# Amandaynzhou/MMT-PSM

Hardware: AMD Instinct MI355X
Metric: imgs/sec (student+teacher step, 1000x1000, AUG_K=2) (higher is better)
Workload: dtype f32

## Files before the change

### include/mmtpsm.h

```cpp
#ifndef MMTPSM_H
#define MMTPSM_H
#include <stdint.h>
#ifdef __cplusplus
extern "C" {
#endif

#define MMT_EINVAL (-22)

int mmt_version(void);

typedef struct {
  const float* feat[4];
  float* grad_feat[4];
  int H[4];
  int W[4];
  float scale[4];
  int num_levels;
  int N;
  int C;
} mmt_pyramid;

int mmt_roi_align_forward(const mmt_pyramid* pyr , const float* rois, const int32_t* levels,
                          int K, int PH, int PW, int sampling_ratio, float* out, void* stream);
int mmt_roi_align_forward_bf16(const mmt_pyramid* pyr , const float* rois, const int32_t* levels,
// ... 132 lines not shown
} mmt_conv_args;

int mmt_conv_forward(const mmt_conv_args* a , void* stream);
enum { MMT_ENTRY_LIB = 0, MMT_ENTRY_F16 = 1 };
enum { MMT_ASSUME_X = 1, MMT_ASSUME_W = 2, MMT_ASSUME_W_PLANES = 4, MMT_ASSUME_X_PLANES = 8, MMT_ASSUME_F16_SCALARS = 16 };
enum {
  MMT_ROUTE_NONE = 0,
  MMT_ROUTE_FP32 = 1,
  MMT_ROUTE_SPLIT = 2,
  MMT_ROUTE_DMA = 3,
  MMT_ROUTE_DMA_BF16X = 4,
  MMT_ROUTE_ROWS = 5,
  MMT_ROUTE_STRIP = 6,
  MMT_ROUTE_PG = 7,
  MMT_ROUTE_C64 = 8
};
enum { MMT_X_AS_IS = 0, MMT_X_BF16_PLANES = 1, MMT_X_F16_PLANES = 2 };
typedef struct {
  int family;
  int tag;
  int bm, bn;
  int kgroups;
  int panels;
  int ksplit;
  int strip_tw, strip_ksplit, strip_korder;
  int pg_rows, pg_ksplit;
  int wanted;
  int x_form;
  int writes_rb;
  int switches;
} mmt_conv_route_t;
int mmt_conv_route(const mmt_conv_args* a , int entry, int assume, mmt_conv_route_t* out );
enum { MMT_SW_SPLITK = 1, MMT_SW_STRIP = 2, MMT_SW_ROWS = 4, MMT_SW_PG = 8, MMT_SW_C64 = 16, MMT_SW_DIRECT_EPI = 32 };
int mmt_conv_switches(void);
int mmt_set_conv_precision(int mode);
int mmt_amax(const float* x, long n, const float* rowscale, long inner, int rows, float* amax , void* stream);
int mmt_amax_stats(const float* x, long n, float* slot , void* stream);
int mmt_sum_stats(const float* a, const float* b, const float* c, const float* d, float* y, long n,
                  float* slot , void* stream);
int mmt_stats_combine(const float* const* slots , int n, float* out , void* stream);
int mmt_split_planes_f16(const float* x, void* planes, long plane_stride, long n, float scale, const float* amax ,
                         float* scale_out , float* amax_next ,
                         float* zero_slot , void* stream);
int mmt_pack_weight_f16(const float* w, void* planes, long plane_stride, int Cout, int K, float scale, const float* amax,
                        float* scale_out, void* stream);
int mmt_pack_weight_flipped_f16(const float* w, const float* scale, void* planes, long plane_stride, int Cout, int KH, int KW,
                                int Cin, const float* amax, float* scale_out, void* stream);
int mmt_conv3x3_strip_f16x2(const mmt_conv_args* a , const float* s_x , const float* s_w , void* stream);
int mmt_conv_forward_f16x2(const mmt_conv_args* a , const float* x_amax , const float* s_w , void* stream);
int mmt_get_conv_precision(void);
int mmt_stem_fused(const float* x, int N, int H, int W, const float* w_s2d, const void* w_planes, long w_plane_stride,
                   const float* s_w , const float* scale, const float* shift, const float* x_slot , float* y,
                   float* y_slot , void* stream);
int mmt_c64_conv3_fused(const float* x, int N, int H, int W, const float* w2, const void* w2_planes, long w2_plane_stride,
                        const float* s_w2 , const float* scale2, const float* shift2, const float* x_slot ,
                        const float* w3, const void* w3_planes, long w3_plane_stride, const float* s_w3 , const float* scale3,
                        const float* shift3, const float* res, float* out, float* out_slot ,
                        const float* o2_scale , int o2_scale_is_amax, float* o2_amax_next ,
                        float* out_amax_next , const float* w1, const void* w1_planes, long w1_plane_stride,
                        const float* s_w1 , const float* scale1, const float* shift1, const float* out_scale ,
                        float* o1_next, float* o1_next_slot , void* stream);
int mmt_conv_wgrad_planes_splits(const mmt_conv_args* a );
int mmt_conv_wgrad_planes(const mmt_conv_args* a , const float* dy, const void* x_planes, long x_plane_stride,
                          const void* dy_planes, long dy_plane_stride, const float* s_x, const float* s_dy, const float* rowscale,
                          float* dw, float* dbias, float* workspace, void* stream);
typedef struct {
  void* fn;
  long a[16];
} mmt_call;
int mmt_replay(const mmt_call* calls , int n, int* failed_index );
int mmt_split_planes_f16_rb(const float* x, void* planes, long plane_stride, int rows, int W, int C, const float* amax,
                            float* scale_out, void* stream);
typedef struct mmt_wgrad_job {
  mmt_conv_args a;
  const float* dy; const float* rowscale; float* dw; float* dbias;
  const void* x_planes; long x_plane_stride; const void* dy_planes; long dy_plane_stride; const float* s_x; const float* s_dy;
} mmt_wgrad_job;
int mmt_conv_wgrad_group_workspace(const mmt_wgrad_job* jobs , int n, long* floats_out );
int mmt_conv_wgrad_group(const mmt_wgrad_job* jobs , int n, float* workspace, long workspace_floats, void* stream);
int mmt_sum_stats_rb(const float* a, const float* b, const float* c, const float* d, float* y, int rows, int W, int C, float* slot,
                     void* planes, long plane_stride, const float* scale, float* amax_next, void* stream);
int mmt_rb_scales_update(float* state, int n, void* stream);
int mmt_conv_forward_pg(const mmt_conv_args* a , const float* s_x , const float* s_w , int tile_rows,
                        int ksplit, void* stream);
typedef struct { long src_off, dst_off; int Cout, K, unit0, pad; } mmt_pack_desc;
long mmt_packed_weight_elems(int Cout, int K);
int mmt_pack_weight(const float* w, void* planes, long plane_stride, int Cout, int K, void* stream);
int mmt_pack_weight_flipped(const float* w, const float* scale, void* planes, long plane_stride, int Cout, int KH, int KW,
                            int Cin, void* stream);
int mmt_split_planes(const float* x, void* planes, long plane_stride, long n, void* stream);
typedef struct { const float* w; const float* scale; void* dst; long plane_stride; int Cout, KH, KW, Cin, unit0, pad; } mmt_flip_desc;
int mmt_pack_weights_flipped(const mmt_flip_desc* descs , const int* unit_desc , int n_units, void* stream);
int mmt_pack_weights(const float* base, void* planes, long plane_stride, const mmt_pack_desc* descs ,
                     const int* unit_desc , int n_units, void* stream);
int mmt_pack_weights_f16(const float* base, void* planes, long plane_stride, const mmt_pack_desc* descs ,
                         const int* unit_desc , int n_units, int n_descs, float* stat , void* stream);
int mmt_pack_weights_flipped_f16(const mmt_flip_desc* descs , const int* unit_desc , int n_units, int n_descs,
                                 float* stat , void* stream);

int mmt_conv_wgrad_splits(const mmt_conv_args* a );
int mmt_conv_wgrad(const mmt_conv_args* a , const float* dy,
                   const float* rowscale , float* dw, float* dbias ,
                   float* workspace , void* stream);

int mmt_colsum(const float* dy, int M, int C, float* out, void* stream);

// ... 116 lines not shown
```

### mmt-psm_amd/csrc/conv_stem.hip

```cpp
#include "conv_shared.h"

namespace {

struct StemP {
  const float* x;
  const unsigned short* wpl; long wpl_stride;
  const float* w;
  const float* scale; const float* shift;
  float* y;
  const float* x_slot;
  const float* s_w;
  unsigned* amax_out; int amax_stats;
  int N, H, W, Hc, Wc, Hp, Wp, tiles_y, tiles_x;
};

constexpr int SPH = 19, SPW = 35, SPIX = SPH * SPW;
constexpr int SPL = 672 * 32;
constexpr int SB_OFF = 2 * SPL;
constexpr int STEM_LDS = 128 * 1024;

__device__ __forceinline__ float stem_exact(const StemP& p, int n, int oy, int ox, int co) {
  float acc = 0.f;
  for (int a = 0; a < 4; a++)
    for (int b = 0; b < 4; b++) {
      const int si = oy - 2 + a, sj = ox - 2 + b;
      if ((unsigned)si >= (unsigned)p.Hc || (unsigned)sj >= (unsigned)p.Wc) continue;
      for (int ch = 0; ch < 16; ch++) {
        const int c = ch & 3;
        if (c == 3) continue;
        const float xv = p.x[(((long)n * 3 + c) * p.H + 2 * si + (ch >> 3)) * p.W + 2 * sj + ((ch >> 2) & 1)];
        acc = fmaf(xv, p.w[((co * 4 + a) * 4 + b) * 16 + ch], acc);
      }
    }
  return acc;
}

__global__ __launch_bounds__(512) void stem_fused_kernel(const StemP p) {
  extern __shared__ __attribute__((aligned(16))) float lds[];
  char* const sm = (char*)lds;
  const int tid = threadIdx.x, lane = tid & 63;
  const int wave = __builtin_amdgcn_readfirstlane(tid >> 6);
  int bid = blockIdx.x;
  const int tx = bid % p.tiles_x; bid /= p.tiles_x;
  const int ty = bid % p.tiles_y;
  const int n = bid / p.tiles_y;
  const int py0 = ty * 7, px0 = tx * 15;
  const int oy0 = 2 * py0 - 1, ox0 = 2 * px0 - 1;
  const int sy0 = oy0 - 2, sx0 = ox0 - 2;
  const F16Guard guard = f16_guard_load(p.x_slot);
  const float sx = f16_scale_of(*p.x_slot);

  if (f16_guard_bad(guard)) {
    float amx = 0.f;
    for (int o = tid; o < 7 * 15 * 64; o += 512) {
      const int co = o & 63, q = (o >> 6) % 15, j = (o >> 6) / 15;
      const int py = py0 + j, px = px0 + q;
      if (py >= p.Hp || px >= p.Wp) continue;
      float m = 0.f;
      for (int dy = -1; dy <= 1; dy++)
        for (int dx = -1; dx <= 1; dx++) {
          const int oy = 2 * py + dy, ox = 2 * px + dx;
          if ((unsigned)oy >= (unsigned)p.Hc || (unsigned)ox >= (unsigned)p.Wc) continue;
          m = fmaxf(m, fmaxf(stem_exact(p, n, oy, ox, co) * p.scale[co] + p.shift[co], 0.f));
        }
      p.y[(((long)n * p.Hp + py) * p.Wp + px) * 64 + co] = m;
      amx = fmaxf(amx, m);
    }
    if (p.amax_out && amx > 0.f) atomicMax(p.amax_out, __builtin_bit_cast(unsigned, amx));
    return;
  }

  {
    const __amdgpu_buffer_rsrc_t rs_b = __builtin_amdgcn_make_buffer_rsrc((void*)p.wpl, 0, 0x7ffffff0, 0x00020000);
#pragma unroll
    for (int i = 0; i < 8; i++) {
      const int item = wave + 8 * i, q = item >> 5, rest = item & 31;
      __builtin_amdgcn_raw_ptr_buffer_load_lds(rs_b, (lds_ptr_t)(sm + SB_OFF + item * 1024), 16,
                                               (int)((q * p.wpl_stride + (long)rest * 512 + lane * 8) * 2), 0, 0, 0);
    }
  }
  typedef float f32x2 __attribute__((ext_vector_type(2)));
#pragma unroll
  for (int rnd = 0; rnd < 3; rnd++) {
    const int item = tid + 512 * rnd;
    if (item < 2 * SPIX) {
      const int pix = item >> 1, bh = item & 1;
      const int pr = pix / SPW, pc = pix - pr * SPW;
      const int si = sy0 + pr, sj = sx0 + pc;
      f32x2 v[3];
      const bool ok = (unsigned)si < (unsigned)p.Hc && (unsigned)sj < (unsigned)p.Wc;
#pragma unroll
      for (int c = 0; c < 3; c++)
        v[c] = ok ? *(const f32x2*)(p.x + (((long)n * 3 + c) * p.H + 2 * si + bh) * p.W + 2 * sj) : f32x2{0.f, 0.f};
      uint2 o0[2], o1[2];
      split4h(f32x4{v[0][0], v[1][0], v[2][0], 0.f}, sx, o0);
      split4h(f32x4{v[0][1], v[1][1], v[2][1], 0.f}, sx, o1);
      char* const dst = sm + pix * 32 + ((bh ^ (pix >> 3)) & 1) * 16;
      *(uint4*)dst = uint4{o0[0].x, o0[0].y, o1[0].x, o1[0].y};
      *(uint4*)(dst + SPL) = uint4{o0[1].x, o0[1].y, o1[1].x, o1[1].y};
    }
  }
  asm volatile("s_waitcnt vmcnt(0) lgkmcnt(0)" ::: "memory");
  __syncthreads();

  const int lr = lane & 31, kh2 = lane >> 5;
  const int boff = SB_OFF + lr * 32 + (((kh2 ^ (lr >> 3)) & 1) << 4);
  auto a_addr = [&](int a, int ta, int tb) {
    const int pidx = (2 * wave + a + ta) * SPW + lr + tb;
    return pidx * 32 + (((kh2 ^ (pidx >> 3)) & 1) << 4);
  };
  f32x16 acc[2][2];
#pragma unroll
  for (int a = 0; a < 2; a++)
#pragma unroll
    for (int b = 0; b < 2; b++)
#pragma unroll
      for (int r = 0; r < 16; r++) acc[a][b][r] = 0.f;
  auto fread = [&](int s, f16x8 (&fa)[2][2], f16x8 (&fb)[2][2]) {
    const int ta = s >> 2, tb = s & 3;
#pragma unroll
    for (int a = 0; a < 2; a++) {
      const int ad = a_addr(a, ta, tb);
      fa[0][a] = *(const f16x8*)(sm + ad);
      fa[1][a] = *(const f16x8*)(sm + ad + SPL);
    }
#pragma unroll
    for (int q = 0; q < 2; q++)
#pragma unroll
      for (int b = 0; b < 2; b++) fb[q][b] = *(const f16x8*)(sm + boff + ((q * 16 + s) * 2 + b) * 1024);
  };
  auto mma = [&](const f16x8 (&fa)[2][2], const f16x8 (&fb)[2][2]) {
#pragma unroll
    for (int pr = 0; pr < 3; pr++) {
      const int qa = pr == 1 ? 1 : 0, qb = pr == 0 ? 1 : 0;
#pragma unroll
      for (int a = 0; a < 2; a++)
#pragma unroll
        for (int b = 0; b < 2; b++)
          acc[a][b] = __builtin_amdgcn_mfma_f32_32x32x16_f16(fa[qa][a], fb[qb][b], acc[a][b], 0, 0, 0);
    }
  };
  {
    f16x8 faP[2][2], fbP[2][2], faQ[2][2], fbQ[2][2];
    fread(0, faP, fbP);
#pragma unroll
    for (int s = 0; s < 16; s += 2) {
      fread(s + 1, faQ, fbQ);
      mma(faP, fbP);
      if (s + 2 < 16) fread(s + 2, faP, fbP);
      mma(faQ, fbQ);
    }
  }
  __syncthreads();

  const int col_l = lane & 31, rq = lane >> 5;
  const float inv = 1.f / (sx * *p.s_w);
  float sc[2], sh[2];
#pragma unroll
  for (int b = 0; b < 2; b++) { sc[b] = p.scale[b * 32 + col_l] * inv; sh[b] = p.shift[b * 32 + col_l]; }
  f32x16 m01[2];
#pragma unroll
  for (int b = 0; b < 2; b++)
#pragma unroll
    for (int r = 0; r < 16; r++) {
      const int ox = ox0 + 8 * (r >> 2) + (r & 3) + 4 * rq;
      const bool cok = (unsigned)ox < (unsigned)p.Wc;
      float v[2];
#pragma unroll
      for (int a = 0; a < 2; a++) {
        const int oy = oy0 + 2 * wave + a;
        const float t = fmaxf(acc[a][b][r] * sc[b] + sh[b], 0.f);
        v[a] = (cok && (unsigned)oy < (unsigned)p.Hc) ? t : 0.f;
      }
      acc[0][b][r] = v[0];
      m01[b][r] = fmaxf(v[0], v[1]);
    }
  float* const xr = lds;
  float* const hv = lds + 8 * 32 * 64;
#pragma unroll
  for (int b = 0; b < 2; b++)
#pragma unroll
    for (int r = 0; r < 16; r++)
      xr[(wave * 32 + 8 * (r >> 2) + (r & 3) + 4 * rq) * 64 + b * 32 + col_l] = acc[0][b][r];
  __syncthreads();
  if (wave < 7) {
#pragma unroll
    for (int b = 0; b < 2; b++)
#pragma unroll
      for (int r = 0; r < 16; r++) {
        const int col = 8 * (r >> 2) + (r & 3) + 4 * rq;
        hv[(wave * 32 + col) * 64 + b * 32 + col_l] = fmaxf(m01[b][r], xr[((wave + 1) * 32 + col) * 64 + b * 32 + col_l]);
      }
  }
  __syncthreads();
  float amx = 0.f, asum = 0.f, acnt = 0.f;
  for (int o = tid; o < 7 * 15 * 16; o += 512) {
    const int c4 = o & 15, q = (o >> 4) % 15, j = (o >> 4) / 15;
    const int py = py0 + j, px = px0 + q;
    if (py >= p.Hp || px >= p.Wp) continue;
    const f32x4* const row = (const f32x4*)(hv + (j * 32 + 2 * q) * 64) + c4;
    const f32x4 t0 = row[0], t1 = row[16], t2 = row[32];
    f32x4 m;
#pragma unroll
    for (int e = 0; e < 4; e++) {
      m[e] = fmaxf(fmaxf(t0[e], t1[e]), t2[e]);
      amx = fmaxf(amx, m[e]);
      asum += m[e];
    }
    acnt += 4.f;
    *(f32x4*)(p.y + (((long)n * p.Hp + py) * p.Wp + px) * 64 + c4 * 4) = m;
  }
  if (p.amax_out) {
    __syncthreads();
    float* const red = lds;
    const bool stats = p.amax_stats && (blockIdx.x & 63) == 0;
#pragma unroll
    for (int o = 32; o > 0; o >>= 1) amx = fmaxf(amx, __shfl_xor(amx, o, 64));
    if (stats) {
#pragma unroll
      for (int o = 32; o > 0; o >>= 1) { asum += __shfl_xor(asum, o, 64); acnt += __shfl_xor(acnt, o, 64); }
    }
    if (lane == 0) { red[wave] = amx; red[16 + wave] = asum; red[32 + wave] = acnt; }
    __syncthreads();
    if (tid == 0) {
      float m = red[0], sm_ = red[16], cn = red[32];
      for (int i = 1; i < 8; i++) { m = fmaxf(m, red[i]); sm_ += red[16 + i]; cn += red[32 + i]; }
      const unsigned bits = __builtin_bit_cast(unsigned, m);
      if (m > 0.f && bits > __hip_atomic_load(p.amax_out, __ATOMIC_RELAXED, __HIP_MEMORY_SCOPE_AGENT)) atomicMax(p.amax_out, bits);
      if (stats && cn > 0.f) {
        const int k = (blockIdx.x >> 6) & 15;
        atomicAdd((float*)p.amax_out + 1 + k, sm_);
        atomicAdd((float*)p.amax_out + 17 + k, cn);
      }
    }
  }
}


struct C64Tail {
  const unsigned short* w3pl; long w3pl_stride;
  const float* w3;
  const float* scale; const float* shift;
  const float* res;
  float* out;
  const float* s_w3;
  const float* s_o2; int s_o2_amax;
  unsigned* o2_amax_next;
  unsigned* amax_out;
  unsigned* out_amax_next;
  const unsigned short* w1pl; long w1pl_stride; const float* w1; const float* scale1; const float* shift1; const float* s_w1;
  const float* s_out; float* o1n; unsigned* amax_o1n;
};
constexpr int C64_PW = 18, C64_PIX = 180, C64_SLAB = 192 * 32, C64_PL = 4 * C64_SLAB, C64_BOFF = 2 * C64_PL;
constexpr int C64_RED = 32768;
constexpr int C64_W1B = 32768;

__device__ __forceinline__ void c64_dma16(const void* g, void* l) {
#if defined(__HIP_DEVICE_COMPILE__)
  const unsigned la = __builtin_amdgcn_readfirstlane((unsigned)(unsigned long)(__attribute__((address_space(3))) char*)l);
  asm volatile("s_mov_b32 m0, %1\n\ts_nop 0\n\tglobal_load_lds_dwordx4 %0, off" ::"v"(g), "s"(la) : "m0", "memory");
#endif
}

__device__ __forceinline__ void c64_tail_exact(const ConvP& p, const C64Tail& t, const float* lds, const int img, const int oy0, const int ox0,
                                               const int wave, const int lane, float& amx, float& asum, float& acnt) {
  const float* const o2 = lds + wave * 2048;
  for (int j = 0; j < 4; j++) {
    const int c = lane + 64 * j;
    const float* const wr = t.w3 + c * 64;
    const float sc = t.scale ? t.scale[c] : 1.f, sh = t.shift ? t.shift[c] : 0.f;
    for (int i = 0; i < 32; i++) {
      const int oy = oy0 + 2 * wave + (i >> 4), ox = ox0 + (i & 15);
      if (oy >= p.Ho || ox >= p.Wo) continue;
      float acc = 0.f;
      for (int k = 0; k < 64; k++) acc = fmaf(o2[i * 64 + k], wr[k], acc);
      const long o = ((long)(img * p.Ho + oy) * p.Wo + ox) * 256 + c;
      float v = acc * sc + sh;
      if (t.res) v += t.res[o];
      v = fmaxf(v, 0.f);
      t.out[o] = v;
      amx = fmaxf(amx, v); asum += v; acnt += 1.f;
    }
  }
}

__device__ __forceinline__ float c64_o2_exact(const ConvP& p, float* lds, const int img, const int oy0, const int ox0, const int wave,
                                              const int lane) {
// ... 487 lines not shown

}

namespace mmtconv {
template <int FUSE>
static int launch_c64_form(const ConvP& p, const C64Tail& t, hipStream_t s) {
  constexpr int LDS = C64_BOFF + 2 * 16384;
  static bool done = false;
  if (!done) {
    const hipError_t e = hipFuncSetAttribute((const void*)conv3x3_c64_kernel<FUSE>, hipFuncAttributeMaxDynamicSharedMemorySize, LDS);
    if (e != hipSuccess) return (int)e;
    done = true;
  }
  const int tiles = p.N * ((p.Ho + 7) >> 3) * ((p.Wo + 15) >> 4);
  hipLaunchKernelGGL(conv3x3_c64_kernel<FUSE>, dim3(tiles), dim3(256), LDS, s, p, t);
  MMT_LAUNCH_CHECK();
  return 0;
}

int launch_c64(const ConvP& p, hipStream_t s) { return launch_c64_form<0>(p, C64Tail{}, s); }
}

extern "C" int mmt_c64_conv3_fused(const float* x, int N, int H, int W, const float* w2, const void* w2_planes, long w2_plane_stride,
                                   const float* s_w2, const float* scale2, const float* shift2, const float* x_slot, const float* w3,
                                   const void* w3_planes, long w3_plane_stride, const float* s_w3, const float* scale3,
                                   const float* shift3, const float* res, float* out, float* out_slot, const float* o2_scale,
                                   int o2_scale_is_amax, float* o2_amax_next, float* out_amax_next, const float* w1,
                                   const void* w1_planes, long w1_plane_stride, const float* s_w1, const float* scale1,
                                   const float* shift1, const float* out_scale, float* o1_next, float* o1_next_slot, void* stream) {
  if (!x || !w2 || !w2_planes || !s_w2 || !x_slot || !w3 || !w3_planes || !s_w3 || !res || !out || !o2_scale || N <= 0 || H <= 0 || W <= 0 ||
      (((size_t)w2_planes | (size_t)w3_planes | (size_t)x) & 15) || ((w2_plane_stride | w3_plane_stride) & 7) ||
      (((size_t)res | (size_t)out) & 3) || precision() != 3)
    return MMT_EINVAL;
  if (w1_planes && (!w1 || !s_w1 || !out_scale || !o1_next || ((size_t)w1_planes & 15) || (w1_plane_stride & 7) || ((size_t)o1_next & 3) ||
                    (const void*)res == (const void*)out))
    return MMT_EINVAL;
  if ((long)N * H * W * 1024 >= (1L << 31)) return MMT_EINVAL;
  ConvP p = {};
  p.x = x; p.w = w2; p.scale = scale2; p.shift = shift2;
  p.N = N; p.H = p.Ho = H; p.W = p.Wo = W; p.Cin = p.Cout = 64; p.KH = p.KW = 3; p.stride = 1; p.pad = 1;
  p.relu = 1; p.out_stride = 1; p.M = N * H * W; p.K = 576; p.cin32 = p.cin4 = 1;
  p.wpl = (const unsigned short*)w2_planes; p.wpl_stride = w2_plane_stride;
  p.f16_sx = x_slot; p.f16_ax = 1; p.f16_sw = s_w2; p.guard_x = x_slot;
  C64Tail t = {};
  t.w3pl = (const unsigned short*)w3_planes; t.w3pl_stride = w3_plane_stride; t.w3 = w3; t.scale = scale3; t.shift = shift3;
  t.res = res; t.out = out; t.s_w3 = s_w3; t.s_o2 = o2_scale; t.s_o2_amax = o2_scale_is_amax ? 1 : 0;
  t.o2_amax_next = (unsigned*)o2_amax_next; t.amax_out = (unsigned*)out_slot; t.out_amax_next = (unsigned*)out_amax_next;
  if (!w1_planes) return launch_c64_form<1>(p, t, (hipStream_t)stream);
  t.w1pl = (const unsigned short*)w1_planes; t.w1pl_stride = w1_plane_stride; t.w1 = w1; t.scale1 = scale1; t.shift1 = shift1;
  t.s_w1 = s_w1; t.s_out = out_scale; t.o1n = o1_next; t.amax_o1n = (unsigned*)o1_next_slot;
  return launch_c64_form<2>(p, t, (hipStream_t)stream);
}

extern "C" int mmt_stem_fused(const float* x, int N, int H, int W, const float* w_s2d, const void* w_planes, long w_plane_stride,
                              const float* s_w, const float* scale, const float* shift, const float* x_slot, float* y, float* y_slot,
                              void* stream) {
  if (!x || !w_s2d || !w_planes || !s_w || !scale || !shift || !x_slot || !y || N <= 0 || H < 8 || W < 8 || (H & 3) || (W & 3) ||
      ((size_t)w_planes & 15) || (w_plane_stride & 7) || ((size_t)x & 7) || ((size_t)y & 15) || precision() != 3)
    return MMT_EINVAL;
  if ((long)N * 3 * H * W >= (1L << 31)) return MMT_EINVAL;
  StemP p;
  p.x = x; p.wpl = (const unsigned short*)w_planes; p.wpl_stride = w_plane_stride; p.w = w_s2d;
  p.scale = scale; p.shift = shift; p.y = y; p.x_slot = x_slot; p.s_w = s_w;
  p.amax_out = (unsigned*)y_slot; p.amax_stats = y_slot ? 1 : 0;
  p.N = N; p.H = H; p.W = W; p.Hc = H / 2; p.Wc = W / 2; p.Hp = H / 4; p.Wp = W / 4;
  p.tiles_y = mmt_cdiv(p.Hp, 7); p.tiles_x = mmt_cdiv(p.Wp, 15);
  static bool done = false;
  if (!done) {
    const hipError_t e = hipFuncSetAttribute((const void*)stem_fused_kernel, hipFuncAttributeMaxDynamicSharedMemorySize, STEM_LDS);
    if (e != hipSuccess) return (int)e;
    done = true;
  }
  hipLaunchKernelGGL(stem_fused_kernel, dim3(N * p.tiles_y * p.tiles_x), dim3(512), STEM_LDS, (hipStream_t)stream, p);
  MMT_LAUNCH_CHECK();
  return 0;
}
```

### mmt-psm_amd/maskrcnn_benchmark/_hip.py

```python
import ctypes
import weakref
import os
import threading as _threading

import torch

_HERE = os.path.dirname(os.path.abspath(__file__))
LIB_PATH = os.path.join(os.path.dirname(_HERE), "libmmtpsm.so")

c_void_p, c_int, c_float, c_double, c_int64 = ctypes.c_void_p, ctypes.c_int, ctypes.c_float, ctypes.c_double, ctypes.c_int64


class Pyramid(ctypes.Structure):
    _fields_ = [("feat", c_void_p * 4), ("grad_feat", c_void_p * 4), ("H", c_int * 4), ("W", c_int * 4),
                ("scale", c_float * 4), ("num_levels", c_int), ("N", c_int), ("C", c_int)]


class RoiMaps(ctypes.Structure):
    _fields_ = [("feat", c_void_p * 4), ("grad_feat", c_void_p * 4), ("H", c_int * 4), ("W", c_int * 4), ("C", c_int * 4),
                ("c_off", c_int * 4), ("scale", c_float * 4), ("num_maps", c_int), ("N", c_int), ("out_C", c_int)]


class ConvArgs(ctypes.Structure):
    _fields_ = [("x", c_void_p), ("w", c_void_p), ("scale", c_void_p), ("shift", c_void_p), ("res", c_void_p),
# ... 93 lines not shown
    "mmt_rpn_post_select": [ctypes.POINTER(RpnPostArgs), c_void_p],
    "mmt_sample_fg_bg": [c_void_p, c_int, c_void_p, c_void_p, c_int, c_int, c_int, c_void_p, c_void_p, c_void_p, c_void_p],
    "mmt_box_decode": [c_void_p, c_void_p, c_int, c_int, c_float, c_float, c_float, c_float, c_float, c_void_p, c_void_p, c_int,
                       c_void_p, c_void_p],
    "mmt_split_planes": [c_void_p, c_void_p, ctypes.c_long, ctypes.c_long, c_void_p],
    "mmt_pack_weights": [c_void_p, c_void_p, ctypes.c_long, c_void_p, c_void_p, c_int, c_void_p],
    "mmt_pack_weights_flipped": [c_void_p, c_void_p, c_int, c_void_p],
    "mmt_pack_weights_f16": [c_void_p, c_void_p, ctypes.c_long, c_void_p, c_void_p, c_int, c_int, c_void_p, c_void_p],
    "mmt_pack_weights_flipped_f16": [c_void_p, c_void_p, c_int, c_int, c_void_p, c_void_p],
    "mmt_pack_weight_flipped": [c_void_p, c_void_p, c_void_p, ctypes.c_long, c_int, c_int, c_int, c_int, c_void_p],
    "mmt_conv_wgrad_splits": [ctypes.POINTER(ConvArgs)],
    "mmt_conv_wgrad": [ctypes.POINTER(ConvArgs), c_void_p, c_void_p, c_void_p, c_void_p, c_void_p, c_void_p],
    "mmt_colsum": [c_void_p, c_int, c_int, c_void_p, c_void_p],
    "mmt_weight_flip_transpose": [c_void_p, c_void_p, c_void_p, c_int, c_int, c_int, c_int, c_void_p],
    "mmt_maxpool3x3s2": [c_void_p, c_void_p, c_int, c_int, c_int, c_int, c_int, c_int, c_void_p],
    "mmt_amax": [c_void_p, ctypes.c_long, c_void_p, ctypes.c_long, c_int, c_void_p, c_void_p],
    "mmt_amax_stats": [c_void_p, ctypes.c_long, c_void_p, c_void_p],
    "mmt_det_postprocess": [c_void_p, c_void_p, c_void_p, c_void_p, c_int, c_int, c_float, c_float, c_int, c_void_p,
                            c_void_p, c_void_p, c_void_p, c_void_p, c_void_p],
    "mmt_position_embedding": [c_void_p, c_int, c_int, c_int, c_void_p, c_void_p, c_void_p],
    "mmt_sample_fg_bg_wide": [c_void_p, c_int, c_void_p, c_void_p, c_int, c_int, c_int, c_int, c_void_p, c_void_p, c_void_p, c_void_p,
                              c_void_p],
    "mmt_rpn_loss": [c_void_p, c_void_p, c_void_p, c_void_p, c_void_p, c_void_p, ctypes.c_long, c_float, c_void_p, c_void_p, c_void_p,
                     c_void_p, c_void_p],
    "mmt_box_loss": [c_void_p, c_void_p, c_void_p, c_void_p, c_int, c_int, c_void_p, c_void_p, c_void_p, c_void_p],
    "mmt_box_loss_rows": [c_void_p, c_void_p, c_void_p, c_void_p, c_int, c_int, c_void_p, c_void_p, c_void_p, c_void_p, c_void_p],
    "mmt_relation_attention_fwd": [c_void_p, c_void_p, c_void_p, c_void_p, c_void_p, c_int, c_int, c_int, c_int, c_int, c_int, c_float,
                                   c_void_p, c_void_p, c_void_p],
    "mmt_relation_attention_bwd": [c_void_p, c_void_p, c_void_p, c_void_p, c_void_p, c_void_p, c_int, c_int, c_int, c_int, c_int, c_float,
                                   c_void_p, c_void_p, c_void_p, c_void_p, c_void_p, c_void_p],
    "mmt_ciam_fwd": [c_void_p, c_void_p, c_int, c_int, c_int, c_int, c_void_p, c_void_p, c_void_p, c_void_p, c_void_p],
    "mmt_ciam_bwd": [c_void_p, c_void_p, c_int, c_int, c_int, c_int, c_void_p, c_void_p, c_void_p, c_void_p, c_void_p, c_void_p,
                     c_void_p, c_void_p, c_void_p],
    "mmt_stats_combine": [c_void_p, c_int, c_void_p, c_void_p],
    "mmt_sum_stats": [c_void_p, c_void_p, c_void_p, c_void_p, c_void_p, ctypes.c_long, c_void_p, c_void_p],
    "mmt_split_planes_f16": [c_void_p, c_void_p, ctypes.c_long, ctypes.c_long, c_float, c_void_p, c_void_p, c_void_p, c_void_p, c_void_p],
    "mmt_split_planes_f16_rb": [c_void_p, c_void_p, ctypes.c_long, c_int, c_int, c_int, c_void_p, c_void_p, c_void_p],
    "mmt_replay": [c_void_p, c_int, c_void_p],
    "mmt_conv_wgrad_group_workspace": [c_void_p, c_int, ctypes.POINTER(ctypes.c_long)],
    "mmt_conv_wgrad_group": [c_void_p, c_int, c_void_p, ctypes.c_long, c_void_p],
    "mmt_sum_stats_rb": [c_void_p, c_void_p, c_void_p, c_void_p, c_void_p, c_int, c_int, c_int, c_void_p, c_void_p, ctypes.c_long, c_void_p,
                         c_void_p, c_void_p],
    "mmt_rb_scales_update": [c_void_p, c_int, c_void_p],
    "mmt_conv_wgrad_planes_splits": [ctypes.POINTER(ConvArgs)],
    "mmt_conv_wgrad_planes": [ctypes.POINTER(ConvArgs), c_void_p, c_void_p, ctypes.c_long, c_void_p, ctypes.c_long, c_void_p, c_void_p,
                              c_void_p, c_void_p, c_void_p, c_void_p, c_void_p],
    "mmt_pack_weight_f16": [c_void_p, c_void_p, ctypes.c_long, c_int, c_int, c_float, c_void_p, c_void_p, c_void_p],
    "mmt_pack_weight_flipped_f16": [c_void_p, c_void_p, c_void_p, ctypes.c_long, c_int, c_int, c_int, c_int, c_void_p, c_void_p, c_void_p],
    "mmt_conv3x3_strip_f16x2": [ctypes.POINTER(ConvArgs), c_void_p, c_void_p, c_void_p],
    "mmt_conv_forward_f16x2": [ctypes.POINTER(ConvArgs), c_void_p, c_void_p, c_void_p],
    "mmt_conv_forward_pg": [ctypes.POINTER(ConvArgs), c_void_p, c_void_p, c_int, c_int, c_void_p],
    "mmt_stem_fused": [c_void_p, c_int, c_int, c_int, c_void_p, c_void_p, ctypes.c_long, c_void_p, c_void_p, c_void_p, c_void_p, c_void_p,
                       c_void_p, c_void_p],
    "mmt_c64_conv3_fused": [c_void_p, c_int, c_int, c_int, c_void_p, c_void_p, ctypes.c_long, c_void_p, c_void_p, c_void_p, c_void_p, c_void_p,
                            c_void_p, ctypes.c_long, c_void_p, c_void_p, c_void_p, c_void_p, c_void_p, c_void_p, c_void_p, c_int, c_void_p,
                            c_void_p, c_void_p, c_void_p, ctypes.c_long, c_void_p, c_void_p, c_void_p, c_void_p, c_void_p, c_void_p,
                            c_void_p],
    "mmt_maxpool3x3s2_bf16": [c_void_p, c_void_p, c_int, c_int, c_int, c_int, c_int, c_int, c_void_p],
    "mmt_gconv3x3_forward": [c_void_p, c_void_p, c_void_p, c_void_p, c_void_p, c_int, c_int, c_int, c_int, c_int, c_int, c_int, c_void_p],
    "mmt_gconv3x3_dgrad": [c_void_p, c_void_p, c_void_p, c_void_p, c_void_p, c_void_p, c_int, c_int, c_int, c_int, c_int, c_int, c_void_p],
    "mmt_gconv3x3_wgrad": [c_void_p, c_void_p, c_void_p, c_void_p, c_int, c_int, c_int, c_int, c_int, c_int, c_void_p],
    "mmt_maxpool3x3s2_backward": [c_void_p, c_void_p, c_void_p, c_int, c_int, c_int, c_int, c_void_p],
    "mmt_stem_wgrad": [c_void_p, c_void_p, c_void_p, c_void_p, c_int, c_int, c_int, c_void_p],
    "mmt_mask_bce": [c_void_p, c_void_p, c_void_p, c_int, c_int, c_int, c_float, c_void_p, c_void_p, c_void_p],
    "mmt_mgd_level_forward": [c_void_p, ctypes.POINTER(MgdTeachers), c_void_p, c_int, c_int, c_int, c_int, c_void_p, c_void_p],
    "mmt_mgd_level_backward": [c_void_p, ctypes.POINTER(MgdTeachers), c_void_p, c_int, c_int, c_int, c_int, c_void_p, c_void_p, c_void_p],
    "mmt_mgd_views_forward": [ctypes.POINTER(MgdStudents), ctypes.POINTER(MgdTeachers), c_void_p, c_int, c_int, c_int, c_int, c_void_p,
                              c_void_p],
    "mmt_mgd_views_backward": [ctypes.POINTER(MgdStudents), ctypes.POINTER(MgdTeachers), c_void_p, c_int, c_int, c_int, c_int, c_void_p,
                               c_void_p, c_void_p],
    "mmt_mask_pool": [c_void_p, c_int, c_int, c_int, c_int, c_int, c_void_p, c_void_p],
    "mmt_psm_rows": [c_void_p, c_int, c_void_p, c_int, c_int, c_void_p, c_float, c_int, c_int, c_void_p, c_void_p, c_void_p],
    "mmt_psm_variance": [c_void_p, c_int, c_int, c_int, c_int, c_void_p, c_void_p],
    "mmt_ema_update": [c_void_p, c_void_p, c_int64, c_double, c_void_p],
    "mmt_sgd_momentum": [c_void_p, c_void_p, c_void_p, c_int64, c_float, c_float, c_float, c_int, c_void_p],
    "mmt_grad_guard": [c_void_p, c_int64, c_void_p, c_void_p, c_float, c_void_p],
    "mmt_sgd_momentum_guarded": [c_void_p, c_void_p, c_void_p, c_int64, c_float, c_float, c_float, c_int, c_void_p, c_void_p],
    "mmt_paste_masks": [c_void_p, c_void_p, c_void_p, c_void_p, c_int, c_int, c_int, c_int, c_int, c_float, c_void_p, c_void_p],
    "mmt_paste_mask_stack": [c_void_p, c_void_p, c_int, c_int, c_int, c_int, c_float, c_void_p, c_void_p],
    "mmt_polygon_targets": [c_void_p, c_void_p, c_void_p, c_void_p, c_int, c_int, c_void_p, c_void_p, c_void_p],
    "mmt_mask_pack": [c_void_p, c_int, c_int, c_int, c_void_p, c_void_p, c_void_p],
    "mmt_paste_mask_words": [c_void_p, c_void_p, c_int, c_int, c_int, c_int, c_float, c_void_p, c_void_p, c_void_p],
    "mmt_mask_expand": [c_void_p, c_void_p, c_int, c_int, c_int, c_void_p, c_void_p, c_void_p],
    "mmt_mask_transition_counts": [c_void_p, c_int, c_int, c_int, c_void_p, c_void_p],
    "mmt_mask_transition_positions": [c_void_p, c_int, c_int, c_int, c_void_p, c_void_p, c_void_p],
    "mmt_mask_pair_intersections": [c_void_p, c_void_p, c_int, c_void_p, c_void_p, c_int, c_int, c_int, c_void_p, c_void_p],
    "mmt_polygon_mask_words_workspace": [c_int, c_int, c_int, c_void_p],
    "mmt_polygon_mask_words": [c_void_p, c_void_p, c_int, c_void_p, c_int, c_int, c_int, c_void_p, ctypes.c_int64, c_void_p, c_void_p,
                               c_void_p],
    "mmt_mask_words_integral": [c_void_p, c_void_p, c_int, c_int, c_int, c_void_p, c_void_p],
    "mmt_mask_words_resample": [c_void_p, c_int, c_int, c_int, c_int, c_int, c_int, c_int, c_int, c_int, c_int, c_void_p, c_void_p,
                                c_void_p],
    "mmt_mask_words_targets": [c_void_p, c_int, c_int, c_int, c_void_p, c_void_p, c_int, c_int, c_void_p, c_void_p],
    "mmt_set_deterministic": [c_int],
    "mmt_get_deterministic": [],
    "mmt_roi_align_backward_ordered": [ctypes.POINTER(Pyramid), c_void_p, c_void_p, c_int, c_int, c_int, c_int, c_void_p, c_int, c_void_p],
    "mmt_colsum_ordered": [c_void_p, c_int, c_int, c_void_p, c_void_p, c_void_p],
    "mmt_stem_wgrad_ordered": [c_void_p, c_void_p, c_void_p, c_void_p, c_int, c_int, c_int, c_void_p, ctypes.c_long, c_void_p],
    "mmt_mask_bce_ordered": [c_void_p, c_void_p, c_void_p, c_int, c_int, c_int, c_float, c_void_p, c_void_p, c_void_p, c_void_p],
    "mmt_mgd_level_forward_ordered": [c_void_p, ctypes.POINTER(MgdTeachers), c_void_p, c_int, c_int, c_int, c_int, c_void_p, c_void_p, c_void_p],
    "mmt_mgd_views_forward_ordered": [ctypes.POINTER(MgdStudents), ctypes.POINTER(MgdTeachers), c_void_p, c_int, c_int, c_int, c_int, c_void_p,
                                      c_void_p, c_void_p],
    "mmt_box_loss_ordered": [c_void_p, c_void_p, c_void_p, c_void_p, c_int, c_int, c_void_p, c_void_p, c_void_p, c_void_p, c_void_p, c_void_p],
    "mmt_ciam_bwd_ordered": [c_void_p, c_void_p, c_int, c_int, c_int, c_int, c_void_p, c_void_p, c_void_p, c_void_p, c_void_p, c_void_p,
                             c_void_p, c_void_p, c_void_p, c_void_p],
}
# ... 2634 lines not shown
```

Measured before the change: 132.5.

## Make stem kernel persistent with double-buffered input patch prefetch

```diff
diff --git a/include/mmtpsm.h b/include/mmtpsm.h
--- a/include/mmtpsm.h
+++ b/include/mmtpsm.h
@@ -208,6 +208,9 @@
 int mmt_stem_fused(const float* x, int N, int H, int W, const float* w_s2d, const void* w_planes, long w_plane_stride,
                    const float* s_w , const float* scale, const float* shift, const float* x_slot , float* y,
                    float* y_slot , void* stream);
+int mmt_stem_fused_blocks(const float* x, int N, int H, int W, const float* w_s2d, const void* w_planes, long w_plane_stride,
+                          const float* s_w , const float* scale, const float* shift, const float* x_slot , float* y,
+                          float* y_slot , int max_blocks, void* stream);
 int mmt_c64_conv3_fused(const float* x, int N, int H, int W, const float* w2, const void* w2_planes, long w2_plane_stride,
                         const float* s_w2 , const float* scale2, const float* shift2, const float* x_slot ,
                         const float* w3, const void* w3_planes, long w3_plane_stride, const float* s_w3 , const float* scale3,
diff --git a/mmt-psm_amd/csrc/conv_stem.hip b/mmt-psm_amd/csrc/conv_stem.hip
--- a/mmt-psm_amd/csrc/conv_stem.hip
+++ b/mmt-psm_amd/csrc/conv_stem.hip
@@ -11,13 +11,23 @@
   const float* x_slot;
   const float* s_w;
   unsigned* amax_out; int amax_stats;
-  int N, H, W, Hc, Wc, Hp, Wp, tiles_y, tiles_x;
+  int N, H, W, Hc, Wc, Hp, Wp, tiles_y, tiles_x, tiles;
 };
 
 constexpr int SPH = 19, SPW = 35, SPIX = SPH * SPW;
 constexpr int SPL = 672 * 32;
-constexpr int SB_OFF = 2 * SPL;
-constexpr int STEM_LDS = 128 * 1024;
+constexpr int SP_OFF = 64 * 1024;
+constexpr int SPBUF = 2 * SPL;
+constexpr int SRED_OFF = SP_OFF + 2 * SPBUF;
+constexpr int STEM_LDS = SRED_OFF + 256;
+static_assert(8 * 32 * 32 * 4 <= SPBUF, "the pooling stage of one 32-channel half fits the consumed patch buffer");
+static_assert(STEM_LDS <= 160 * 1024, "one CU's LDS");
+
+struct StemTile { int n, py0, px0; };
+__device__ __forceinline__ StemTile stem_tile(const StemP& p, int t) {
+  const int tx = t % p.tiles_x; t /= p.tiles_x;
+  return StemTile{t / p.tiles_y, (t % p.tiles_y) * 7, tx * 15};
+}
 
 __device__ __forceinline__ float stem_exact(const StemP& p, int n, int oy, int ox, int co) {
   float acc = 0.f;
@@ -40,33 +50,31 @@
   char* const sm = (char*)lds;
   const int tid = threadIdx.x, lane = tid & 63;
   const int wave = __builtin_amdgcn_readfirstlane(tid >> 6);
-  int bid = blockIdx.x;
-  const int tx = bid % p.tiles_x; bid /= p.tiles_x;
-  const int ty = bid % p.tiles_y;
-  const int n = bid / p.tiles_y;
-  const int py0 = ty * 7, px0 = tx * 15;
-  const int oy0 = 2 * py0 - 1, ox0 = 2 * px0 - 1;
-  const int sy0 = oy0 - 2, sx0 = ox0 - 2;
+  const int nblk = gridDim.x;
   const F16Guard guard = f16_guard_load(p.x_slot);
   const float sx = f16_scale_of(*p.x_slot);
 
   if (f16_guard_bad(guard)) {
-    float amx = 0.f;
-    for (int o = tid; o < 7 * 15 * 64; o += 512) {
-      const int co = o & 63, q = (o >> 6) % 15, j = (o >> 6) / 15;
-      const int py = py0 + j, px = px0 + q;
-      if (py >= p.Hp || px >= p.Wp) continue;
-      float m = 0.f;
-      for (int dy = -1; dy <= 1; dy++)
-        for (int dx = -1; dx <= 1; dx++) {
-          const int oy = 2 * py + dy, ox = 2 * px + dx;
-          if ((unsigned)oy >= (unsigned)p.Hc || (unsigned)ox >= (unsigned)p.Wc) continue;
-          m = fmaxf(m, fmaxf(stem_exact(p, n, oy, ox, co) * p.scale[co] + p.shift[co], 0.f));
-        }
-      p.y[(((long)n * p.Hp + py) * p.Wp + px) * 64 + co] = m;
-      amx = fmaxf(amx, m);
-    }
-    if (p.amax_out && amx > 0.f) atomicMax(p.amax_out, __builtin_bit_cast(unsigned, amx));
+#pragma unroll 1
+    for (int t = blockIdx.x; t < p.tiles; t += nblk) {
+      const StemTile tl = stem_tile(p, t);
+      float amx = 0.f;
+      for (int o = tid; o < 7 * 15 * 64; o += 512) {
+        const int co = o & 63, q = (o >> 6) % 15, j = (o >> 6) / 15;
+        const int py = tl.py0 + j, px = tl.px0 + q;
+        if (py >= p.Hp || px >= p.Wp) continue;
+        float m = 0.f;
+        for (int dy = -1; dy <= 1; dy++)
+          for (int dx = -1; dx <= 1; dx++) {
+            const int oy = 2 * py + dy, ox = 2 * px + dx;
+            if ((unsigned)oy >= (unsigned)p.Hc || (unsigned)ox >= (unsigned)p.Wc) continue;
+            m = fmaxf(m, fmaxf(stem_exact(p, tl.n, oy, ox, co) * p.scale[co] + p.shift[co], 0.f));
+          }
+        p.y[(((long)tl.n * p.Hp + py) * p.Wp + px) * 64 + co] = m;
+        amx = fmaxf(amx, m);
+      }
+      if (p.amax_out && amx > 0.f) atomicMax(p.amax_out, __builtin_bit_cast(unsigned, amx));
+    }
     return;
   }
 
@@ -75,164 +83,199 @@
 #pragma unroll
     for (int i = 0; i < 8; i++) {
       const int item = wave + 8 * i, q = item >> 5, rest = item & 31;
-      __builtin_amdgcn_raw_ptr_buffer_load_lds(rs_b, (lds_ptr_t)(sm + SB_OFF + item * 1024), 16,
+      __builtin_amdgcn_raw_ptr_buffer_load_lds(rs_b, (lds_ptr_t)(sm + item * 1024), 16,
                                                (int)((q * p.wpl_stride + (long)rest * 512 + lane * 8) * 2), 0, 0, 0);
     }
   }
   typedef float f32x2 __attribute__((ext_vector_type(2)));
-#pragma unroll
-  for (int rnd = 0; rnd < 3; rnd++) {
-    const int item = tid + 512 * rnd;
-    if (item < 2 * SPIX) {
+  auto patch_ok = [&](const StemTile& tl, int item) {
+    const int pix = item >> 1;
+    const int pr = pix / SPW, pc = pix - pr * SPW;
+    const int si = 2 * tl.py0 - 3 + pr, sj = 2 * tl.px0 - 3 + pc;
+    return item < 2 * SPIX && (unsigned)si < (unsigned)p.Hc && (unsigned)sj < (unsigned)p.Wc;
+  };
+  auto patch_request = [&](const StemTile& tl, f32x2 (&v)[3][3]) {
+    const long plane = (long)p.H * p.W;
+#pragma unroll
+    for (int rnd = 0; rnd < 3; rnd++) {
+      const int item = tid + 512 * rnd;
       const int pix = item >> 1, bh = item & 1;
       const int pr = pix / SPW, pc = pix - pr * SPW;
-      const int si = sy0 + pr, sj = sx0 + pc;
-      f32x2 v[3];
-      const bool ok = (unsigned)si < (unsigned)p.Hc && (unsigned)sj < (unsigned)p.Wc;
-#pragma unroll
-      for (int c = 0; c < 3; c++)
-        v[c] = ok ? *(const f32x2*)(p.x + (((long)n * 3 + c) * p.H + 2 * si + bh) * p.W + 2 * sj) : f32x2{0.f, 0.f};
-      uint2 o0[2], o1[2];
-      split4h(f32x4{v[0][0], v[1][0], v[2][0], 0.f}, sx, o0);
-      split4h(f32x4{v[0][1], v[1][1], v[2][1], 0.f}, sx, o1);
-      char* const dst = sm + pix * 32 + ((bh ^ (pix >> 3)) & 1) * 16;
-      *(uint4*)dst = uint4{o0[0].x, o0[0].y, o1[0].x, o1[0].y};
-      *(uint4*)(dst + SPL) = uint4{o0[1].x, o0[1].y, o1[1].x, o1[1].y};
-    }
-  }
+      const int si = 2 * tl.py0 - 3 + pr, sj = 2 * tl.px0 - 3 + pc;
+      const bool ok = patch_ok(tl, item);
+      const float* const src = ok ? p.x + ((long)tl.n * 3 * p.H + 2 * si + bh) * p.W + 2 * sj : p.x;
+      const long cs = ok ? plane : 0;
+#pragma unroll
+      for (int c = 0; c < 3; c++) v[rnd][c] = *(const f32x2*)(src + c * cs);
+    }
+  };
+  auto patch_commit = [&](const StemTile& tl, const f32x2 (&v)[3][3], int buf, int rnd) {
+    const int item = tid + 512 * rnd;
+    const int pix = item < 2 * SPIX ? item >> 1 : 671, bh = item & 1;
+    const bool ok = patch_ok(tl, item);
+    f32x2 u[3];
+#pragma unroll
+    for (int c = 0; c < 3; c++) u[c] = ok ? v[rnd][c] : f32x2{0.f, 0.f};
+    uint2 o0[2], o1[2];
+    split4h(f32x4{u[0][0], u[1][0], u[2][0], 0.f}, sx, o0);
+    split4h(f32x4{u[0][1], u[1][1], u[2][1], 0.f}, sx, o1);
+    char* const dst = sm + buf + pix * 32 + ((bh ^ (pix >> 3)) & 1) * 16;
+    *(uint4*)dst = uint4{o0[0].x, o0[0].y, o1[0].x, o1[0].y};
+    *(uint4*)(dst + SPL) = uint4{o0[1].x, o0[1].y, o1[1].x, o1[1].y};
+  };
+  static_assert(SPIX <= 671 && (18 * SPW + 34) < SPIX, "pixel 671 is padding: the last fragment read is pixel 664");
+  StemTile tl = stem_tile(p, blockIdx.x);
+  f32x2 pv[3][3];
+  patch_request(tl, pv);
+#pragma unroll
+  for (int rnd = 0; rnd < 3; rnd++) patch_commit(tl, pv, SP_OFF, rnd);
   asm volatile("s_waitcnt vmcnt(0) lgkmcnt(0)" ::: "memory");
   __syncthreads();
 
   const int lr = lane & 31, kh2 = lane >> 5;
-  const int boff = SB_OFF + lr * 32 + (((kh2 ^ (lr >> 3)) & 1) << 4);
-  auto a_addr = [&](int a, int ta, int tb) {
-    const int pidx = (2 * wave + a + ta) * SPW + lr + tb;
-    return pidx * 32 + (((kh2 ^ (pidx >> 3)) & 1) << 4);
-  };
-  f32x16 acc[2][2];
-#pragma unroll
-  for (int a = 0; a < 2; a++)
-#pragma unroll
-    for (int b = 0; b < 2; b++)
-#pragma unroll
-      for (int r = 0; r < 16; r++) acc[a][b][r] = 0.f;
-  auto fread = [&](int s, f16x8 (&fa)[2][2], f16x8 (&fb)[2][2]) {
-    const int ta = s >> 2, tb = s & 3;
-#pragma unroll
-    for (int a = 0; a < 2; a++) {
-      const int ad = a_addr(a, ta, tb);
-      fa[0][a] = *(const f16x8*)(sm + ad);
-      fa[1][a] = *(const f16x8*)(sm + ad + SPL);
-    }
-#pragma unroll
-    for (int q = 0; q < 2; q++)
-#pragma unroll
-      for (int b = 0; b < 2; b++) fb[q][b] = *(const f16x8*)(sm + boff + ((q * 16 + s) * 2 + b) * 1024);
-  };
-  auto mma = [&](const f16x8 (&fa)[2][2], const f16x8 (&fb)[2][2]) {
-#pragma unroll
-    for (int pr = 0; pr < 3; pr++) {
-      const int qa = pr == 1 ? 1 : 0, qb = pr == 0 ? 1 : 0;
-#pragma unroll
-      for (int a = 0; a < 2; a++)
-#pragma unroll
-        for (int b = 0; b < 2; b++)
-          acc[a][b] = __builtin_amdgcn_mfma_f32_32x32x16_f16(fa[qa][a], fb[qb][b], acc[a][b], 0, 0, 0);
-    }
-  };
-  {
-    f16x8 faP[2][2], fbP[2][2], faQ[2][2], fbQ[2][2];
-    fread(0, faP, fbP);
-#pragma unroll
-    for (int s = 0; s < 16; s += 2) {
-      fread(s + 1, faQ, fbQ);
-      mma(faP, fbP);
-      if (s + 2 < 16) fread(s + 2, faP, fbP);
-      mma(faQ, fbQ);
-    }
-  }
-  __syncthreads();
-
+  const int boff = lr * 32 + (((kh2 ^ (lr >> 3)) & 1) << 4);
   const int col_l = lane & 31, rq = lane >> 5;
   const float inv = 1.f / (sx * *p.s_w);
   float sc[2], sh[2];
 #pragma unroll
   for (int b = 0; b < 2; b++) { sc[b] = p.scale[b * 32 + col_l] * inv; sh[b] = p.shift[b * 32 + col_l]; }
-  f32x16 m01[2];
-#pragma unroll
-  for (int b = 0; b < 2; b++)
-#pragma unroll
-    for (int r = 0; r < 16; r++) {
-      const int ox = ox0 + 8 * (r >> 2) + (r & 3) + 4 * rq;
-      const bool cok = (unsigned)ox < (unsigned)p.Wc;
-      float v[2];
+  float bmax = 0.f;
+  int cur = SP_OFF;
+
+#pragma unroll 1
+  for (int t = blockIdx.x; t < p.tiles; t += nblk, cur = SP_OFF + SPBUF - (cur - SP_OFF)) {
+    const int py0 = tl.py0, px0 = tl.px0, n = tl.n;
+    const int oy0 = 2 * py0 - 1, ox0 = 2 * px0 - 1;
+    const StemTile tn = stem_tile(p, t + nblk < p.tiles ? t + nblk : t);
+    const int nxt = SP_OFF + SPBUF - (cur - SP_OFF);
+    patch_request(tn, pv);
+    __builtin_amdgcn_sched_barrier(0);
+
+    auto a_addr = [&](int a, int ta, int tb) {
+      const int pidx = (2 * wave + a + ta) * SPW + lr + tb;
+      return cur + pidx * 32 + (((kh2 ^ (pidx >> 3)) & 1) << 4);
+    };
+    f32x16 acc[2][2];
+#pragma unroll
+    for (int a = 0; a < 2; a++)
+#pragma unroll
+      for (int b = 0; b < 2; b++)
+#pragma unroll
+        for (int r = 0; r < 16; r++) acc[a][b][r] = 0.f;
+    auto fread = [&](int s, f16x8 (&fa)[2][2], f16x8 (&fb)[2][2]) {
+      const int ta = s >> 2, tb = s & 3;
 #pragma unroll
       for (int a = 0; a < 2; a++) {
-        const int oy = oy0 + 2 * wave + a;
-        const float t = fmaxf(acc[a][b][r] * sc[b] + sh[b], 0.f);
-        v[a] = (cok && (unsigned)oy < (unsigned)p.Hc) ? t : 0.f;
-      }
-      acc[0][b][r] = v[0];
-      m01[b][r] = fmaxf(v[0], v[1]);
-    }
-  float* const xr = lds;
-  float* const hv = lds + 8 * 32 * 64;
-#pragma unroll
-  for (int b = 0; b < 2; b++)
-#pragma unroll
-    for (int r = 0; r < 16; r++)
-      xr[(wave * 32 + 8 * (r >> 2) + (r & 3) + 4 * rq) * 64 + b * 32 + col_l] = acc[0][b][r];
-  __syncthreads();
-  if (wave < 7) {
-#pragma unroll
-    for (int b = 0; b < 2; b++)
+        const int ad = a_addr(a, ta, tb);
+        fa[0][a] = *(const f16x8*)(sm + ad);
+        fa[1][a] = *(const f16x8*)(sm + ad + SPL);
+      }
+#pragma unroll
+      for (int q = 0; q < 2; q++)
+#pragma unroll
+        for (int b = 0; b < 2; b++) fb[q][b] = *(const f16x8*)(sm + boff + ((q * 16 + s) * 2 + b) * 1024);
+    };
+    auto mma = [&](const f16x8 (&fa)[2][2], const f16x8 (&fb)[2][2]) {
+#pragma unroll
+      for (int pr = 0; pr < 3; pr++) {
+        const int qa = pr == 1 ? 1 : 0, qb = pr == 0 ? 1 : 0;
+#pragma unroll
+        for (int a = 0; a < 2; a++)
+#pragma unroll
+          for (int b = 0; b < 2; b++)
+            acc[a][b] = __builtin_amdgcn_mfma_f32_32x32x16_f16(fa[qa][a], fb[qb][b], acc[a][b], 0, 0, 0);
+      }
+    };
+    {
+      f16x8 faP[2][2], fbP[2][2], faQ[2][2], fbQ[2][2];
+      fread(0, faP, fbP);
+#pragma unroll
+      for (int s = 0; s < 16; s += 2) {
+        fread(s + 1, faQ, fbQ);
+        mma(faP, fbP);
+        if (s + 2 < 16) fread(s + 2, faP, fbP);
+        mma(faQ, fbQ);
+        if (s == 4 || s == 8 || s == 12) {
+          __builtin_amdgcn_sched_barrier(0);
+          patch_commit(tn, pv, nxt, s / 4 - 1);
+        }
+      }
+    }
+    __syncthreads();
+
+    float* const xr = (float*)(sm + cur);
+    float amx = 0.f, asum = 0.f, acnt = 0.f;
+#pragma unroll
+    for (int b = 0; b < 2; b++) {
+      float m01[16];
+      if (b) __syncthreads();
 #pragma unroll
       for (int r = 0; r < 16; r++) {
         const int col = 8 * (r >> 2) + (r & 3) + 4 * rq;
-        hv[(wave * 32 + col) * 64 + b * 32 + col_l] = fmaxf(m01[b][r], xr[((wave + 1) * 32 + col) * 64 + b * 32 + col_l]);
-      }
-  }
-  __syncthreads();
-  float amx = 0.f, asum = 0.f, acnt = 0.f;
-  for (int o = tid; o < 7 * 15 * 16; o += 512) {
-    const int c4 = o & 15, q = (o >> 4) % 15, j = (o >> 4) / 15;
-    const int py = py0 + j, px = px0 + q;
-    if (py >= p.Hp || px >= p.Wp) continue;
-    const f32x4* const row = (const f32x4*)(hv + (j * 32 + 2 * q) * 64) + c4;
-    const f32x4 t0 = row[0], t1 = row[16], t2 = row[32];
-    f32x4 m;
-#pragma unroll
-    for (int e = 0; e < 4; e++) {
-      m[e] = fmaxf(fmaxf(t0[e], t1[e]), t2[e]);
-      amx = fmaxf(amx, m[e]);
-      asum += m[e];
-    }
-    acnt += 4.f;
-    *(f32x4*)(p.y + (((long)n * p.Hp + py) * p.Wp + px) * 64 + c4 * 4) = m;
-  }
-  if (p.amax_out) {
+        const bool cok = (unsigned)(ox0 + col) < (unsigned)p.Wc;
+        float v[2];
+#pragma unroll
+        for (int a = 0; a < 2; a++) {
+          const int oy = oy0 + 2 * wave + a;
+          const float e = fmaxf(acc[a][b][r] * sc[b] + sh[b], 0.f);
+          v[a] = (cok && (unsigned)oy < (unsigned)p.Hc) ? e : 0.f;
+        }
+        xr[(wave * 32 + col) * 32 + col_l] = v[0];
+        m01[r] = fmaxf(v[0], v[1]);
+      }
+      __syncthreads();
+      if (wave < 7) {
+#pragma unroll
+        for (int r = 0; r < 16; r++) {
+          float* const w = xr + ((wave + 1) * 32 + 8 * (r >> 2) + (r & 3) + 4 * rq) * 32 + col_l;
+          *w = fmaxf(m01[r], *w);
+        }
+      }
+      __syncthreads();
+      for (int o = tid; o < 7 * 15 * 8; o += 512) {
+        const int c4 = o & 7, q = (o >> 3) % 15, j = (o >> 3) / 15;
+        const int py = py0 + j, px = px0 + q;
+        if (py >= p.Hp || px >= p.Wp) continue;
+        const f32x4* const row = (const f32x4*)(xr + ((j + 1) * 32 + 2 * q) * 32) + c4;
+        const f32x4 t0 = row[0], t1 = row[8], t2 = row[16];
+        f32x4 m;
+#pragma unroll
+        for (int e = 0; e < 4; e++) {
+          m[e] = fmaxf(fmaxf(t0[e], t1[e]), t2[e]);
+          amx = fmaxf(amx, m[e]);
+          asum += m[e];
+        }
+        acnt += 4.f;
+        *(f32x4*)(p.y + (((long)n * p.Hp + py) * p.Wp + px) * 64 + b * 32 + c4 * 4) = m;
+      }
+    }
+    float* const red = (float*)(sm + SRED_OFF);
+    const bool stats = p.amax_stats && (t & 63) == 0;
+    if (p.amax_out) {
+#pragma unroll
+      for (int o = 32; o > 0; o >>= 1) amx = fmaxf(amx, __shfl_xor(amx, o, 64));
+      if (stats) {
+#pragma unroll
+        for (int o = 32; o > 0; o >>= 1) { asum += __shfl_xor(asum, o, 64); acnt += __shfl_xor(acnt, o, 64); }
+      }
+      if (lane == 0) { red[wave] = amx; red[16 + wave] = asum; red[32 + wave] = acnt; }
+    }
     __syncthreads();
-    float* const red = lds;
-    const bool stats = p.amax_stats && (blockIdx.x & 63) == 0;
-#pragma unroll
-    for (int o = 32; o > 0; o >>= 1) amx = fmaxf(amx, __shfl_xor(amx, o, 64));
-    if (stats) {
-#pragma unroll
-      for (int o = 32; o > 0; o >>= 1) { asum += __shfl_xor(asum, o, 64); acnt += __shfl_xor(acnt, o, 64); }
-    }
-    if (lane == 0) { red[wave] = amx; red[16 + wave] = asum; red[32 + wave] = acnt; }
-    __syncthreads();
-    if (tid == 0) {
+    if (p.amax_out && tid == 0) {
       float m = red[0], sm_ = red[16], cn = red[32];
       for (int i = 1; i < 8; i++) { m = fmaxf(m, red[i]); sm_ += red[16 + i]; cn += red[32 + i]; }
-      const unsigned bits = __builtin_bit_cast(unsigned, m);
-      if (m > 0.f && bits > __hip_atomic_load(p.amax_out, __ATOMIC_RELAXED, __HIP_MEMORY_SCOPE_AGENT)) atomicMax(p.amax_out, bits);
+      bmax = fmaxf(bmax, m);
       if (stats && cn > 0.f) {
-        const int k = (blockIdx.x >> 6) & 15;
+        const int k = (t >> 6) & 15;
         atomicAdd((float*)p.amax_out + 1 + k, sm_);
         atomicAdd((float*)p.amax_out + 17 + k, cn);
       }
     }
+    tl = tn;
+  }
+  if (p.amax_out && tid == 0) {
+    const unsigned bits = __builtin_bit_cast(unsigned, bmax);
+    if (bmax > 0.f && bits > __hip_atomic_load(p.amax_out, __ATOMIC_RELAXED, __HIP_MEMORY_SCOPE_AGENT)) atomicMax(p.amax_out, bits);
   }
 }
 
@@ -826,11 +869,11 @@
   return launch_c64_form<2>(p, t, (hipStream_t)stream);
 }
 
-extern "C" int mmt_stem_fused(const float* x, int N, int H, int W, const float* w_s2d, const void* w_planes, long w_plane_stride,
-                              const float* s_w, const float* scale, const float* shift, const float* x_slot, float* y, float* y_slot,
-                              void* stream) {
+extern "C" int mmt_stem_fused_blocks(const float* x, int N, int H, int W, const float* w_s2d, const void* w_planes, long w_plane_stride,
+                                     const float* s_w, const float* scale, const float* shift, const float* x_slot, float* y,
+                                     float* y_slot, int max_blocks, void* stream) {
   if (!x || !w_s2d || !w_planes || !s_w || !scale || !shift || !x_slot || !y || N <= 0 || H < 8 || W < 8 || (H & 3) || (W & 3) ||
-      ((size_t)w_planes & 15) || (w_plane_stride & 7) || ((size_t)x & 7) || ((size_t)y & 15) || precision() != 3)
+      ((size_t)w_planes & 15) || (w_plane_stride & 7) || ((size_t)x & 7) || ((size_t)y & 15) || max_blocks < 0 || precision() != 3)
     return MMT_EINVAL;
   if ((long)N * 3 * H * W >= (1L << 31)) return MMT_EINVAL;
   StemP p;
@@ -839,13 +882,28 @@
   p.amax_out = (unsigned*)y_slot; p.amax_stats = y_slot ? 1 : 0;
   p.N = N; p.H = H; p.W = W; p.Hc = H / 2; p.Wc = W / 2; p.Hp = H / 4; p.Wp = W / 4;
   p.tiles_y = mmt_cdiv(p.Hp, 7); p.tiles_x = mmt_cdiv(p.Wp, 15);
-  static bool done = false;
-  if (!done) {
-    const hipError_t e = hipFuncSetAttribute((const void*)stem_fused_kernel, hipFuncAttributeMaxDynamicSharedMemorySize, STEM_LDS);
+  const long tiles = (long)N * p.tiles_y * p.tiles_x;
+  if (tiles >= (1L << 31)) return MMT_EINVAL;
+  p.tiles = (int)tiles;
+  static int cus = 0;
+  if (!cus) {
+    int dev = 0, n = 0;
+    hipError_t e = hipGetDevice(&dev);
+    if (e == hipSuccess) e = hipDeviceGetAttribute(&n, hipDeviceAttributeMultiprocessorCount, dev);
+    if (e == hipSuccess) e = hipFuncSetAttribute((const void*)stem_fused_kernel, hipFuncAttributeMaxDynamicSharedMemorySize, STEM_LDS);
     if (e != hipSuccess) return (int)e;
-    done = true;
-  }
-  hipLaunchKernelGGL(stem_fused_kernel, dim3(N * p.tiles_y * p.tiles_x), dim3(512), STEM_LDS, (hipStream_t)stream, p);
+    if (n <= 0) return MMT_EINVAL;
+    cus = n;
+  }
+  int grid = p.tiles < cus ? p.tiles : cus;
+  if (max_blocks && max_blocks < grid) grid = max_blocks;
+  hipLaunchKernelGGL(stem_fused_kernel, dim3(grid), dim3(512), STEM_LDS, (hipStream_t)stream, p);
   MMT_LAUNCH_CHECK();
   return 0;
 }
+
+extern "C" int mmt_stem_fused(const float* x, int N, int H, int W, const float* w_s2d, const void* w_planes, long w_plane_stride,
+                              const float* s_w, const float* scale, const float* shift, const float* x_slot, float* y, float* y_slot,
+                              void* stream) {
+  return mmt_stem_fused_blocks(x, N, H, W, w_s2d, w_planes, w_plane_stride, s_w, scale, shift, x_slot, y, y_slot, 0, stream);
+}
diff --git a/mmt-psm_amd/maskrcnn_benchmark/_hip.py b/mmt-psm_amd/maskrcnn_benchmark/_hip.py
--- a/mmt-psm_amd/maskrcnn_benchmark/_hip.py
+++ b/mmt-psm_amd/maskrcnn_benchmark/_hip.py
@@ -169,6 +169,8 @@
     "mmt_conv_forward_pg": [ctypes.POINTER(ConvArgs), c_void_p, c_void_p, c_int, c_int, c_void_p],
     "mmt_stem_fused": [c_void_p, c_int, c_int, c_int, c_void_p, c_void_p, ctypes.c_long, c_void_p, c_void_p, c_void_p, c_void_p, c_void_p,
                        c_void_p, c_void_p],
+    "mmt_stem_fused_blocks": [c_void_p, c_int, c_int, c_int, c_void_p, c_void_p, ctypes.c_long, c_void_p, c_void_p, c_void_p, c_void_p,
+                              c_void_p, c_void_p, c_int, c_void_p],
     "mmt_c64_conv3_fused": [c_void_p, c_int, c_int, c_int, c_void_p, c_void_p, ctypes.c_long, c_void_p, c_void_p, c_void_p, c_void_p, c_void_p,
                             c_void_p, ctypes.c_long, c_void_p, c_void_p, c_void_p, c_void_p, c_void_p, c_void_p, c_void_p, c_int, c_void_p,
                             c_void_p, c_void_p, c_void_p, ctypes.c_long, c_void_p, c_void_p, c_void_p, c_void_p, c_void_p, c_void_p,
```

Result: no change. 132.0 (-0.4%).
